# Lingeng56/conformer-pytorch-lightning

Measured on AMD Instinct MI355X. Metric: encoder frames/sec (80-d fbank, T=1000), whole job, higher is better.
Workload: dtype bf16

## Files before the change

### conformer-pytorch-lightning_amd/cfm/__init__.py

```python
import ctypes
import os
import threading

import torch

_HERE = os.path.dirname(os.path.abspath(__file__))
LIB_PATH = os.path.join(os.path.dirname(_HERE), "libconformer_gfx950.so")

F32, BF16, F16 = 0, 1, 2
ACT_NONE, ACT_SILU, ACT_RELU, ACT_GLU, ACT_DSILU, ACT_DRELU = 0, 1, 2, 3, 4, 5
TILE_AUTO_TRAIN = -1

_DT = {torch.float32: F32, torch.bfloat16: BF16, torch.float16: F16}
_TORCH_DT = {F32: torch.float32, BF16: torch.bfloat16, F16: torch.float16}

c_p = ctypes.c_void_p
c_i64 = ctypes.c_int64
c_i32 = ctypes.c_int32
c_f = ctypes.c_float


class GemmDesc(ctypes.Structure):
    _fields_ = [("A", c_p), ("W", c_p), ("W_lo", c_p), ("bias", c_p), ("residual", c_p), ("row_mask", c_p), ("C", c_p),
                ("lda", c_i64), ("ldc", c_i64), ("ldr", c_i64),
# ... 86 lines not shown
                ("p_hidden_m", ctypes.c_float), ("p_hidden", ctypes.c_float), ("p_branch", ctypes.c_float), ("p_attn", ctypes.c_float),
                ("p_attn_out", ctypes.c_float), ("seed", ctypes.c_uint32), ("deterministic", c_i32), ("grads_accumulate", c_i32),
                ("n_groups", c_i32), ("groups", ctypes.POINTER(TrainGroup)), ("defer_wgrad", c_i32)]


_TRAIN_SAVED = ["xn1", "z1", "h1", "xn2", "qkv", "ctx", "xn3", "u", "glu", "s", "xn4", "z2", "h2", "x1", "x2", "x3", "x4", "c", "lse", "stats"]
_TRAIN_SCRATCH = ["dxn", "dz", "dyb", "ds", "dglu", "du", "dctx", "dqkv", "delta", "ln_ws", "dwbn_ws", "dy_ws", "dz2", "dyb2", "dyb3", "dyb4"]
_TRAIN_GRADS = ["slab", "ln_ffm_g", "ln_ffm_b", "ln_mha_g", "ln_mha_b", "ln_conv_g", "ln_conv_b", "ln_ff_g", "ln_ff_b", "ln_final_g", "ln_final_b",
                "ffm_w1", "ffm_b1", "ffm_w2", "ffm_b2", "ff_w1", "ff_b1", "ff_w2", "ff_b2", "out_w", "out_b", "pw2_w", "pw2_b", "dw_w", "dw_b", "bn_g", "bn_b",
                "pos_bias_u", "q_bias", "qkv_row_off", "qkv_bias_off", "pw1_row_off", "pw1_bias_off", "qkv_bias_off2"]


class LayerTrainSaved(ctypes.Structure):
    _fields_ = [(n, c_p) for n in _TRAIN_SAVED]


class LayerTrainScratch(ctypes.Structure):
    _fields_ = [(n, c_p) for n in _TRAIN_SCRATCH]


class LayerTrainGrads(ctypes.Structure):
    _fields_ = [(n, c_p) for n in _TRAIN_GRADS]


class LayerWeights(ctypes.Structure):
    _fields_ = [(n, c_p) for n in _LAYER_W_FIELDS]


class CtcGroup(ctypes.Structure):
    _fields_ = [("logits", c_p), ("ld", c_i64), ("B", c_i32), ("T", c_i32), ("Umax", c_i32), ("enc_lens", c_p), ("labels", c_p), ("label_lens", c_p),
                ("work", c_p), ("alpha", c_p), ("lse", c_p), ("nll", c_p), ("nll_shifted", c_p), ("beta", c_p)]


class RnntDesc(ctypes.Structure):
    _fields_ = [("logits", c_p), ("ld", c_i64), ("logits_dtype", c_i32), ("B", c_i32), ("T", c_i32), ("U1", c_i32), ("V", c_i32), ("blank", c_i32),
                ("targets", c_p), ("logit_lens", c_p), ("target_lens", c_p),
                ("lse", c_p), ("lp_blank", c_p), ("lp_label", c_p), ("alpha", c_p), ("beta", c_p), ("shift", c_p),
                ("nll", c_p), ("nll_shifted", c_p), ("ll_alpha", c_p),
                ("grad", c_p), ("ld_grad", c_i64), ("grad_dtype", c_i32), ("grad_cols", c_i32), ("gscale", ctypes.c_float),
                ("gscale_stride", c_i32), ("gscale_dev", c_p), ("clamp", ctypes.c_float)]


class Lattice(ctypes.Structure):
    _fields_ = [("B", c_i32), ("T_max", c_i32), ("U1_max", c_i32), ("M", c_i64), ("off", c_p), ("T", c_p), ("U", c_p), ("enc_row0", c_p),
                ("pred_row0", c_p), ("n_enc", c_i64), ("n_pred", c_i64), ("blk_off", c_p)]


class RnntPackedDesc(ctypes.Structure):
    _fields_ = [("lat", Lattice), ("logits", c_p), ("ld", c_i64), ("logits_dtype", c_i32), ("V", c_i32), ("blank", c_i32), ("ld_targets", c_i32),
                ("targets", c_p), ("lse", c_p), ("lp_blank", c_p), ("lp_label", c_p), ("alpha", c_p), ("beta", c_p), ("shift", c_p),
                ("nll", c_p), ("nll_shifted", c_p), ("ll_alpha", c_p),
                ("grad", c_p), ("ld_grad", c_i64), ("grad_dtype", c_i32), ("grad_cols", c_i32), ("gscale", ctypes.c_float),
                ("gscale_stride", c_i32), ("gscale_dev", c_p), ("clamp", ctypes.c_float)]


class LnBwdDesc(ctypes.Structure):
    _fields_ = [("x", c_p), ("dy", c_p), ("gamma", c_p), ("row_mask", c_p), ("dres", c_p), ("dx", c_p), ("dgamma", c_p), ("dbeta", c_p), ("ws", c_p),
                ("dx2", c_p), ("M", c_i64), ("D", c_i32), ("dy_dtype", c_i32), ("dx2_dtype", c_i32), ("accumulate", c_i32),
                ("eps", ctypes.c_float), ("alpha2", ctypes.c_float), ("p1", ctypes.c_float), ("p2", ctypes.c_float),
                ("seed1", ctypes.c_uint32), ("seed2", ctypes.c_uint32), ("dx2_row_mask", c_p),
                ("chain_x", c_p), ("chain_gamma", c_p), ("chain_dgamma", c_p), ("chain_dbeta", c_p)]


class GreedyDesc(ctypes.Structure):
    _fields_ = [("embed", c_p), ("lstm_w", c_p * 4), ("lstm_b", c_p * 4), ("proj_w", c_p), ("proj_b", c_p), ("pf_w", c_p), ("pf_b", c_p), ("out_w", c_p),
                ("out_b", c_p), ("enc_proj", c_p), ("token", c_p), ("t", c_p), ("count", c_p), ("frame_count", c_p), ("hyps", c_p), ("lens", c_p),
                ("h", c_p), ("c", c_p), ("h_new", c_p), ("c_new", c_p), ("pred", c_p), ("act", c_p), ("pmax", c_p), ("pidx", c_p), ("done", c_p),
                ("n_done", c_p), ("hyp_cap", c_i64), ("hyp_ld", c_i64), ("B", c_i32), ("T", c_i32), ("L", c_i32), ("E", c_i32), ("H", c_i32),
                ("P", c_i32), ("J", c_i32), ("Vp", c_i32), ("blank", c_i32), ("n_steps", c_i32)]


class GreedyChunkDesc(ctypes.Structure):
    _fields_ = ([("embed", c_p), ("lstm_w", c_p * 4), ("lstm_b", c_p * 4)] +
                [(n, c_p) for n in ("proj_w", "proj_b", "pf_w", "pf_b", "out_w", "out_b", "ef_w", "ef_b", "enc", "enc_proj", "token", "t", "count", "frame_count",
                                    "hyps", "lens", "h", "c", "h_new", "c_new", "pred", "pp", "act", "pmax", "pidx", "rows", "row_off", "row_cnt", "n_rows",
                                    "steps", "overflow", "done", "n_done")] +
                [("hyp_cap", c_i64), ("hyp_ld", c_i64)] +
                [(n, c_i32) for n in ("B", "chunk", "L", "E", "H", "P", "J", "D", "Vp", "blank", "n_steps", "carry")])


class FbankDesc(ctypes.Structure):
    _fields_ = ([(n, c_p) for n in ("samples", "lengths", "feats_length", "carry_in", "carry_out", "fresh_in", "pos_in", "fresh_out", "pos_out", "twiddle", "window",
                                    "mel_w", "mel_start", "mel_len", "mel_off", "out")] + [("ld", c_i64)] +
                [(n, c_i32) for n in ("B", "n_cols", "rows", "F", "win", "shift", "padded", "mel_nnz", "samples_i16", "carry_n", "hop")] +
                [("dither", c_f), ("seed", ctypes.c_uint32)])


class FfnSplitDesc(ctypes.Structure):
    _fields_ = [("x", c_p), ("psum", c_p), ("psum_b2", c_p), ("psum_splits", c_i32), ("psum_alpha", c_f), ("ln1_g", c_p), ("ln1_b", c_p), ("ln2_g", c_p),
                ("ln2_b", c_p), ("rows_out", c_p), ("rows2_out", c_p), ("ln_g", c_p), ("ln_b", c_p), ("w1", c_p), ("b1", c_p), ("N1", c_i32), ("act", c_i32),
                ("w2", c_p), ("psum_out", c_p), ("out16", c_p), ("ldo", c_i64), ("M", c_i32), ("D", c_i32), ("mode", c_i32), ("w_dtype", c_i32), ("eps", c_f),
                ("kv_ring", c_p), ("ring_offsets", c_p), ("ring_T", c_i32), ("ring_H", c_i32), ("ring_Tq", c_i32)]


class LayerScratch(ctypes.Structure):
    _fields_ = [(n, c_p) for n in ("xn", "hid", "qkv", "pos", "ctx", "glu", "dw")] + [("psum", c_p), ("psum_splits", c_i32)]


class LayerIO(ctypes.Structure):
    _fields_ = [("B", c_i32), ("T", c_i32), ("D", c_i32), ("H", c_i32), ("FF", c_i32), ("ktaps", c_i32),
                ("act_dtype", c_i32), ("w_dtype", c_i32),
                ("attn_mask", c_p), ("am_sb", c_i64), ("am_sq", c_i64),
                ("pad_valid", c_p), ("pos_embed", c_p), ("pos_rows", c_i32),
                ("pos_proj", c_p), ("pos_proj_ld", c_i64),
                ("attn_cache", c_p), ("cache_T", c_i32), ("new_cache", c_p), ("after_g", c_p), ("after_b", c_p), ("after_out", c_p),
                ("kv_ring", c_p), ("stream_offset", c_p), ("ring_T", c_i32), ("causal_conv", c_i32), ("conv_cache", c_p), ("pos_shared", c_i32),
                ("next_w", c_p), ("next_x_out", c_p), ("macaron_done", c_i32)]


_lib = None
_lock = threading.Lock()


def lib():
    global _lib
    if _lib is not None:
        return _lib
    with _lock:
        if _lib is not None:
            return _lib
        if not os.path.exists(LIB_PATH):
            raise RuntimeError(
                "libconformer_gfx950.so not found at %s -- build it with `python -c 'import __graft_entry__ as g; g.build()'` "
                "or `make -C conformer-pytorch-lightning_amd/csrc`. There is no CPU fallback." % LIB_PATH)
        L = ctypes.CDLL(LIB_PATH)
        L.cfm_version.restype = ctypes.c_int
        L.cfm_last_error.restype = ctypes.c_char_p
        L.cfm_device_ok.restype = ctypes.c_int
        L.cfm_gemm.argtypes = [ctypes.POINTER(GemmDesc), c_p]
        L.cfm_attention.argtypes = [ctypes.POINTER(AttnDesc), c_p]
        L.cfm_ffn_fused.argtypes = [ctypes.POINTER(FfnDesc), c_p]
        L.cfm_rowchain.argtypes = [ctypes.POINTER(RowChainDesc), c_p]
        L.cfm_rowchain_supported.argtypes = [c_i32, c_i32]
        L.cfm_rowchain_pair_supported.argtypes = [c_i32, c_i32]
        L.cfm_layernorm.argtypes = [c_p, c_p, c_p, c_p, c_i32, c_p, c_p, c_p, c_i32, c_p, ctypes.c_float, c_i64, c_i32, c_p]
        L.cfm_kv_cache_pack.argtypes = [c_p, c_i32, c_p, c_p, c_i32, c_i64, c_i64, c_i64, c_i64, c_p, c_i32, c_i32, c_i32, c_i32, c_p]
        L.cfm_dwconv_bn_silu.argtypes = [c_p, c_i32, c_p, c_p, c_p, c_p, c_p, c_i32, c_i32, c_i32, c_i32, c_i32, c_p]
        L.cfm_conv1_relu.argtypes = [c_p, c_p, c_p, c_p, c_i32, c_i32, c_i32, c_i32, c_i32, c_p, c_p, c_p]
        L.cfm_conv1_relu_mma.argtypes = [c_p, c_p, c_p, c_p, c_i32, c_i32, c_i32, c_i32, c_i32, c_p, c_p, c_p]
        L.cfm_conv12_supported.argtypes = [c_i32, c_i32]
        L.cfm_pack_matrices.argtypes = [c_p, c_i32, c_i64, c_i32, c_i32, c_p]
        L.cfm_pack_vectors.argtypes = [c_p, c_p, c_p, c_i64, c_p]
        L.cfm_greedy_step.argtypes = [ctypes.POINTER(GreedyDesc), c_p]
        L.cfm_greedy_chunk_begin.argtypes = [ctypes.POINTER(GreedyChunkDesc), c_p]
        L.cfm_greedy_chunk_step.argtypes = [ctypes.POINTER(GreedyChunkDesc), c_p]
        L.cfm_fbank.argtypes = [ctypes.POINTER(FbankDesc), c_p]
        L.cfm_fbank_stream.argtypes = [ctypes.POINTER(FbankDesc), c_p]
        L.cfm_ffn_split.argtypes = [ctypes.POINTER(FfnSplitDesc), c_p]
        L.cfm_ffn_split_supported.argtypes = [c_i32, c_i32]
        L.cfm_attention_bwd_force_general.argtypes = [c_i32]
        L.cfm_attention_bwd_force_general.restype = None
        L.cfm_set_cin_merge.argtypes = [c_i32]
        L.cfm_set_cin_merge.restype = c_i32
        L.cfm_dwconv_bn_train_bwd_acc.argtypes = [c_p, c_i32, c_p, c_p, c_p, c_i32, c_p, c_p, c_i32, c_p, c_p, c_p, c_p, c_p, c_p, c_i32, c_i32, c_i32, c_i32, c_i32, c_p]
        L.cfm_layernorm_bwd_fused.argtypes = [ctypes.POINTER(LnBwdDesc), c_p]
        L.cfm_conv12_relu.argtypes = [c_p, c_p, c_p, c_p, c_p, c_p, c_i32, c_i32, c_i32, c_i32, c_i32, c_p, c_p, c_p]
        L.cfm_valid_mask.argtypes = [c_p, c_i32, c_p, c_i32, c_i32, c_i32, c_i32, c_p]
        L.cfm_chunk_mask.argtypes = [c_p, c_i32, c_i32, c_i32, c_p]
        L.cfm_attn_mask.argtypes = [c_p, c_p, c_p, c_i32, c_i32, c_p]
        L.cfm_cast.argtypes = [c_p, c_i32, c_p, c_i32, c_i64, c_p]
        L.cfm_add_rows.argtypes = [c_p, c_p, c_i64, c_i32, c_i32, c_p]
        L.cfm_encoder_layer_forward.argtypes = [ctypes.POINTER(LayerWeights), ctypes.POINTER(LayerScratch),
                                                ctypes.POINTER(LayerIO), c_p, c_p, c_i32, c_p, c_p, c_p]
        L.cfm_ctc_nll.argtypes = [c_p, c_i64, c_i32, c_i32, c_i32, c_p, c_p, c_i32, c_p, c_p, c_p, c_p]
        L.cfm_joint_act.argtypes = [c_p, c_i64, c_p, c_i64, c_p, c_i32, c_i32, c_i32, c_i32, c_i32, c_p]
        L.cfm_joint_act_bwd.argtypes = [c_p, c_i64, c_p, c_i64, c_p, c_p, c_p, c_p, c_i32, c_i32, c_i32, c_i32, c_p]
        L.cfm_joint_act_bwd_ws.argtypes = [c_i32, c_i32, c_i32, c_i32]
        L.cfm_rnnt_nll.argtypes = [ctypes.POINTER(RnntDesc), c_p]
        L.cfm_rnnt_grad.argtypes = [ctypes.POINTER(RnntDesc), c_p]
        L.cfm_rnnt_packed_nll.argtypes = [ctypes.POINTER(RnntPackedDesc), c_p]
        L.cfm_rnnt_packed_grad.argtypes = [ctypes.POINTER(RnntPackedDesc), c_p]
        L.cfm_joint_act_packed.argtypes = [c_p, c_i64, c_p, c_i64, c_p, c_i32, ctypes.POINTER(Lattice), c_i32, c_p]
        L.cfm_joint_act_packed_bwd.argtypes = [c_p, c_i64, c_p, c_i64, c_p, c_p, c_p, c_p, ctypes.POINTER(Lattice), c_i32, c_p]
        c_f = ctypes.c_float
        L.cfm_gemm_tn.argtypes = [ctypes.POINTER(GemmTnDesc), c_p]
        L.cfm_gemm_tn_group.argtypes = [ctypes.POINTER(GemmTnDesc), c_i32, c_p]
        L.cfm_attention_bwd.argtypes = [ctypes.POINTER(AttnBwdDesc), c_p]
        L.cfm_layernorm_bwd_ws.argtypes = [c_i64, c_i32]
        L.cfm_layernorm_bwd.argtypes = [c_p, c_p, c_i32, c_p, c_p, c_p, c_p, c_p, c_p, c_p, c_f, c_i64, c_i32, c_p]
        L.cfm_glu_bwd.argtypes = [c_p, c_i32, c_p, c_i32, c_p, c_i32, c_i64, c_i32, c_p]
        L.cfm_dwconv_bn_ws.argtypes = [c_i32, c_i32, c_i32]
        L.cfm_dwconv_bn_train.argtypes = [c_p, c_i32, c_p, c_p, c_p, c_p, c_p, c_p, c_f, c_f, c_p, c_p, c_p, c_i32, c_p, c_i32, c_i32, c_i32, c_i32, c_p]
        L.cfm_dwconv_bn_train_bwd.argtypes = [c_p, c_i32, c_p, c_p, c_p, c_i32, c_p, c_p, c_i32, c_p, c_p, c_p, c_p, c_p, c_p, c_i32, c_i32, c_i32, c_i32, c_p]
        L.cfm_col2im_relu_bwd.argtypes = [c_p, c_i32, c_p, c_i32, c_p, c_i32, c_i32, c_i32, c_i32, c_i32, c_p]
        L.cfm_conv1_wgrad_ws.argtypes = [c_i32, c_i32, c_i32]
        L.cfm_conv1_wgrad.argtypes = [c_p, c_i32, c_p, c_p, c_p, c_p, c_p, c_p, c_i32, c_i32, c_i32, c_i32, c_p]
        L.cfm_ctc_nll_train_groups.argtypes = [ctypes.POINTER(CtcGroup), c_i32, c_i32, c_p]
        L.cfm_ctc_grad.argtypes = [c_p, c_i64, c_i32, c_i32, c_i32, c_p, c_p, c_i32, c_p, c_p, c_p, c_p, c_p, c_p, c_f, c_p, c_p, c_p]
        L.cfm_adam_step.argtypes = [c_p, c_p, c_p, c_p, c_i64, c_f, c_f, c_f, c_f, c_f, c_i64, c_p, c_p]
        L.cfm_sumsq.argtypes = [c_p, c_i64, c_p, c_i32, c_p, c_p]
        L.cfm_adam_clip_step.argtypes = [c_p, c_p, c_p, c_p, c_i64, c_f, c_f, c_f, c_f, c_f, c_i64, c_p, c_f, c_f, c_i32, c_p, c_p]
        L.cfm_dropout_rows.argtypes = [c_p, c_i32, c_p, c_i32, c_p, c_f, c_f, ctypes.c_uint32, c_f, ctypes.c_uint32, c_i64, c_i32, c_p]
        L.cfm_dropout_mask.argtypes = [c_p, c_i64, c_f, ctypes.c_uint32, c_p]
        L.cfm_encoder_train_forward.argtypes = [c_i32, ctypes.POINTER(LayerTrainWeights), ctypes.POINTER(LayerTrainIO), ctypes.POINTER(LayerTrainSaved),
                                                ctypes.POINTER(LayerTrainScratch), ctypes.POINTER(c_p), c_p]
        L.cfm_encoder_train_backward.argtypes = [c_i32, ctypes.POINTER(LayerTrainWeights), ctypes.POINTER(LayerTrainIO), ctypes.POINTER(LayerTrainSaved),
                                                 ctypes.POINTER(LayerTrainScratch), ctypes.POINTER(LayerTrainGrads), ctypes.POINTER(c_p), c_p, c_p, c_p,
                                                 LAYER_DONE_FN, c_p, ctypes.POINTER(c_p), c_p]
        L.cfm_stream_prep.argtypes = [c_p, c_i32, c_i32, c_i32, c_i32, c_p, c_i32, c_i32, c_p, c_p, c_p, c_p]
        L.cfm_kv_ring_write.argtypes = [c_p, c_p, c_i32, c_i64, c_i64, c_i64, c_i64, c_p, c_p, c_i32, c_i32, c_i32, c_i32, c_i32, c_p]
        L.cfm_stream_advance.argtypes = [c_p, c_p, c_i32, c_i32, c_p]
        L.cfm_dwconv_causal_bn_silu.argtypes = [c_p, c_i32, c_p, c_p, c_p, c_p, c_p, c_p, c_i32, c_i32, c_i32, c_i32, c_i32, c_p]
        L.cfm_conv_cache_update.argtypes = [c_p, c_i32, c_p, c_i32, c_i32, c_i32, c_i32, c_p]
        for name in ("cfm_layernorm_bwd_ws", "cfm_dwconv_bn_ws", "cfm_conv1_wgrad_ws", "cfm_joint_act_bwd_ws"):
            getattr(L, name).restype = c_i64
        L.cfm_prof_enable.argtypes = [c_i32]
        L.cfm_prof_enable.restype = None
        L.cfm_prof_reset.restype = None
        L.cfm_prof_collect.restype = ctypes.c_int
        L.cfm_prof_entry.argtypes = [c_i32, ctypes.c_char_p, c_i32, ctypes.POINTER(c_i64), ctypes.POINTER(ctypes.c_double),
                                     ctypes.POINTER(ctypes.c_double), ctypes.POINTER(ctypes.c_double)]
        for name in ("cfm_gemm", "cfm_ffn_fused", "cfm_rowchain", "cfm_rowchain_supported", "cfm_attention", "cfm_layernorm", "cfm_kv_cache_pack", "cfm_dwconv_bn_silu", "cfm_conv1_relu", "cfm_conv1_relu_mma", "cfm_conv12_relu", "cfm_conv12_supported",
                     "cfm_valid_mask", "cfm_chunk_mask", "cfm_attn_mask", "cfm_cast", "cfm_add_rows",
                     "cfm_encoder_layer_forward", "cfm_ctc_nll", "cfm_joint_act", "cfm_joint_act_bwd", "cfm_rnnt_nll", "cfm_rnnt_grad", "cfm_prof_entry", "cfm_gemm_tn", "cfm_gemm_tn_group", "cfm_attention_bwd",
                     "cfm_layernorm_bwd", "cfm_glu_bwd", "cfm_dwconv_bn_train", "cfm_dwconv_bn_train_bwd", "cfm_col2im_relu_bwd", "cfm_conv1_wgrad",
                     "cfm_ctc_nll_train_groups", "cfm_ctc_grad", "cfm_adam_step", "cfm_adam_clip_step", "cfm_sumsq", "cfm_dropout_rows", "cfm_dropout_mask", "cfm_pack_matrices", "cfm_pack_vectors", "cfm_greedy_step", "cfm_greedy_chunk_begin", "cfm_greedy_chunk_step", "cfm_fbank", "cfm_fbank_stream", "cfm_ffn_split", "cfm_ffn_split_supported", "cfm_layernorm_bwd_fused", "cfm_dwconv_bn_train_bwd_acc",
                     "cfm_encoder_train_forward", "cfm_encoder_train_backward", "cfm_stream_prep", "cfm_kv_ring_write", "cfm_stream_advance", "cfm_dwconv_causal_bn_silu", "cfm_conv_cache_update"):
            getattr(L, name).restype = ctypes.c_int
        _lib = L
    return _lib


def check(rc, what):
    if rc != 0:
        raise RuntimeError("%s failed (status %d): %s" % (what, rc, lib().cfm_last_error().decode(errors="replace")))


def dt_code(t):
    try:
        return _DT[t.dtype if isinstance(t, torch.Tensor) else t]
    except KeyError:
        raise TypeError("cfm: unsupported dtype %s (float32, bfloat16, float16 only)" % (t.dtype if isinstance(t, torch.Tensor) else t))


def torch_dtype(code):
    return _TORCH_DT[code]


def require_hip(*tensors):
    for t in tensors:
        if t is None:
            continue
        if not t.is_cuda:
            raise RuntimeError("cfm: tensor on %s -- this framework runs on MI355X (HIP) only; there is no CPU path" % t.device)


def ptr(t):
    return None if t is None else t.data_ptr()


def stream():
    return torch.cuda.current_stream().cuda_stream


class Precision:

    def __init__(self, name):
        if name not in ("bf16", "fp16", "fp32"):
            raise ValueError("precision must be bf16, fp16 or fp32, got %r" % (name,))
        self.name = name
        self.split = name == "fp32"
        self.w_code = F16 if name == "fp16" else BF16
        self.act_code = F32 if self.split else self.w_code
        self.w_dtype = torch_dtype(self.w_code)
        self.act_dtype = torch_dtype(self.act_code)

    def __repr__(self):
        return "Precision(%s)" % self.name


_precision = Precision(os.environ.get("CFM_PRECISION", "bf16"))


def set_precision(name):
    global _precision
    _precision = name if isinstance(name, Precision) else Precision(name)
    return _precision


def get_precision():
    return _precision


def resolve_precision(module=None):
    p = getattr(module, "precision", None) if module is not None else None
    if p is None:
        return _precision
    return p if isinstance(p, Precision) else Precision(p)


_warned = set()


def check_mode(module, what):
    if module.training:
        return True
    if torch.is_grad_enabled() and what not in _warned and any(q.requires_grad for q in module.parameters()):
        _warned.add(what)
        import warnings
        warnings.warn("%s: eval-mode forward runs inference kernels; its output is detached from the parameters. "
                      "Call .train() for a differentiable forward, or wrap inference in torch.no_grad()." % what)
    return False


from .ops import *
```

### conformer-pytorch-lightning_amd/csrc/frontend.hip

```cpp
#include <string>
#include <type_traits>

#include "cfm_common.h"

namespace {

typedef unsigned int u32x2_a4 __attribute__((ext_vector_type(2), aligned(4)));

#define CFM_INL __attribute__((always_inline))

struct Conv12Args {
    const float* x;
    const float* w1;
    const float* b1;
    const u16* W;
    const float* b2;
    u16* y;
    const float* cm_mean;
    const float* cm_istd;
    int T, F, C, T2, F2, M;
    int m_begin, m_end;
};

template <typename HT, int FM>
__global__ __launch_bounds__(512) void cfm_conv12_kernel(const Conv12Args g) {
    constexpr int BM = 32 * FM, BN = 256, BK = 64;
    constexpr int OPA = BM * (BK / 8), OPW = BN * (BK / 8);
    constexpr int BUF = OPA + OPW;
    constexpr int FN = 4;
    constexpr int NU = 2 * FM;
    constexpr int U = (NU + 7) / 8;
    __shared__ u32x4 smem[2 * BUF + 1024];
    u32x2* const w1tab = (u32x2*)(smem + 2 * BUF);

    const int tid = threadIdx.x, lane = tid & 63;
    const int wave = __builtin_amdgcn_readfirstlane(tid >> 6);
    const int wr = wave >> 2, wc = wave & 3;
    const int l15 = lane & 15, kg = lane >> 4;
    const int m0 = g.m_begin + blockIdx.x * BM;
    const int n0 = blockIdx.y * BN;
    const int N = g.C, K = 9 * g.C;
    const int slabs = g.C >> 6;

    for (int e = tid; e < slabs * 4 * 64; e += 512) {
        const int ln = e & 63, j = (e >> 6) & 3, cs = e >> 8;
        const int r = ln & 15, q = ln >> 4;
        const int ch = cs * 64 + 16 * (r >> 2) + 4 * j + (r & 3);
        u32x2 v = (u32x2){0u, 0u};
        if (q < 3) {
            const float a = g.w1[(3 * q) * g.C + ch], b = g.w1[(3 * q + 1) * g.C + ch], c = g.w1[(3 * q + 2) * g.C + ch];
            v.x = pack2<HT>(a, b);
            v.y = pack2<HT>(c, 0.f);
        } else {
            const float bv = g.b1[ch];
            const float hi = HT::to_f32(HT::from_f32(bv));
            v.x = pack2<HT>(hi, bv - hi);
        }
        w1tab[e] = v;
    }

    unsigned w_off[4];
#pragma unroll
    for (int i = 0; i < 4; ++i) {
        const int r = (i * 8 + wave) * 8 + (lane >> 3);
        const int c = (lane & 7) ^ ((r >> 1) & 7);
        const int n = n0 + r < N ? n0 + r : N - 1;
        w_off[i] = ((unsigned)n * (unsigned)K + c * 8) * 2u;
    }
    auto stageW = [&](int buf, int kt) CFM_INL {
        const unsigned kw = (unsigned)(kt * BK) * 2u;
        u32x4* const Ws = smem + buf * BUF + OPA;
#pragma unroll
        for (int i = 0; i < 4; ++i)
            __builtin_amdgcn_global_load_lds((const __attribute__((address_space(1))) void*)((const char*)g.W + (w_off[i] + kw)),
                                             (__attribute__((address_space(3))) void*)(Ws + (i * 8 + wave) * 64), 16, 0, 0);
    };

    int xbase[U], fcol[U];
#pragma unroll
    for (int ui = 0; ui < U; ++ui) {
        const int u = wave + 8 * ui;
        int m = m0 + u * 16 + l15;
        m = m < g.M ? m : g.M - 1;
        const int per_b = g.T2 * g.F2;
        const int b = m / per_b;
        const int q = m - b * per_b;
        const int t2 = q / g.F2;
        const int f2 = q - t2 * g.F2;
        fcol[ui] = 4 * f2;
        xbase[ui] = (b * g.T + 4 * t2 + (kg < 3 ? kg : 0)) * g.F + 4 * f2;
    }
    float xraw[U][3];
    auto fetch = [&](int tap) CFM_INL {
        const int dt = tap / 3, df = tap - 3 * dt;
#pragma unroll
        for (int ui = 0; ui < U; ++ui) {
            const float* xr = g.x + (xbase[ui] + 2 * dt * g.F + 2 * df);
            float v0 = xr[0], v1 = xr[1], v2 = xr[2];
            if (g.cm_mean) {
                const int f = fcol[ui] + 2 * df;
                v0 -= g.cm_mean[f]; v1 -= g.cm_mean[f + 1]; v2 -= g.cm_mean[f + 2];
                if (g.cm_istd) { v0 *= g.cm_istd[f]; v1 *= g.cm_istd[f + 1]; v2 *= g.cm_istd[f + 2]; }
            }
            xraw[ui][0] = v0; xraw[ui][1] = v1; xraw[ui][2] = v2;
        }
    };
    u32x4 xcur[U];
    auto convert = [&]() CFM_INL {
#pragma unroll
        for (int ui = 0; ui < U; ++ui) {
            xcur[ui] = (u32x4){0u, 0u, 0u, 0u};
            if (kg < 3) {
                xcur[ui].x = pack2<HT>(xraw[ui][0], xraw[ui][1]);
                xcur[ui].y = pack2<HT>(xraw[ui][2], 0.f);
            } else {
                xcur[ui].x = pack2<HT>(1.0f, 1.0f);
            }
        }
    };
    const f32x4 zero4 = (f32x4){0.f, 0.f, 0.f, 0.f};
    auto produce = [&](int buf, int cs) CFM_INL {
        u32x4* const As = smem + buf * BUF;
        u32x4 wf[4];
#pragma unroll
        for (int j = 0; j < 4; ++j) {
            const u32x2 t = w1tab[(cs * 4 + j) * 64 + lane];
            wf[j] = (u32x4){t.x, t.y, 0u, 0u};
        }
#pragma unroll
        for (int ui = 0; ui < U; ++ui) {
            const int u = wave + 8 * ui;
            if (u < NU) {
                f32x4 a[4];
#pragma unroll
                for (int j = 0; j < 4; ++j) {
                    a[j] = HT::mfma(wf[j], xcur[ui], zero4);
                    a[j].x = fmaxf(a[j].x, 0.f); a[j].y = fmaxf(a[j].y, 0.f); a[j].z = fmaxf(a[j].z, 0.f); a[j].w = fmaxf(a[j].w, 0.f);
                }
                const int row = u * 16 + l15;
                const int sw = (row >> 1) & 7;
                As[row * 8 + ((2 * kg) ^ sw)] = pack8<HT>(a[0], a[1]);
                As[row * 8 + ((2 * kg + 1) ^ sw)] = pack8<HT>(a[2], a[3]);
            }
        }
    };

    f32x4 acc[FM][FN];
#pragma unroll
    for (int i = 0; i < FM; ++i)
#pragma unroll
        for (int j = 0; j < FN; ++j) acc[i][j] = zero4;
    const int sw = (lane >> 1) & 7;
    const int a_row = wr * (16 * FM) + l15, w_row = wc * 64 + l15;
    auto compute = [&](int buf) CFM_INL {
        const u32x4* const As = smem + buf * BUF;
        const u32x4* const Ws = As + OPA;
#pragma unroll
        for (int kk = 0; kk < BK / 32; ++kk) {
            const int c = (kk * 4 + kg) ^ sw;
            u32x4 af[FM], wf[FN];
#pragma unroll
            for (int j = 0; j < FN; ++j) wf[j] = Ws[(w_row + j * 16) * 8 + c];
#pragma unroll
            for (int i = 0; i < FM; ++i) af[i] = As[(a_row + i * 16) * 8 + c];
            __builtin_amdgcn_s_setprio(1);
#pragma unroll
            for (int i = 0; i < FM; ++i)
#pragma unroll
                for (int j = 0; j < FN; ++j) acc[i][j] = HT::mfma(wf[j], af[i], acc[i][j]);
            __builtin_amdgcn_s_setprio(0);
        }
    };

    fetch(0);
    stageW(0, 0);
    convert();
    fetch(1);
    __syncthreads();
    produce(0, 0);
    const int q4 = kg * 4;
    f32x4 bias_r[FN];
#pragma unroll
    for (int j = 0; j < FN; ++j) {
        const int col = n0 + wc * 64 + j * 16 + q4;
        bias_r[j] = col + 3 < N ? *(const f32x4*)(g.b2 + col) : zero4;
    }
    __syncthreads();
    for (int tap = 0; tap < 9; ++tap) {
#pragma unroll
        for (int cs = 0; cs < 8; ++cs) {
            if (cs < slabs) {
                const int kt = tap * slabs + cs;
                const int cur = kt & 1;
                const bool last_slab = cs == slabs - 1;
                if (!(tap == 8 && last_slab)) {
                    stageW(cur ^ 1, kt + 1);
                    if (!last_slab) {
                        produce(cur ^ 1, cs + 1);
                    } else {
                        convert();
                        if (tap + 2 < 9) fetch(tap + 2);
                        produce(cur ^ 1, 0);
                    }
                }
                compute(cur);
                __syncthreads();
            }
        }
    }

    const int col0 = n0 + wc * 64 + q4;
#pragma unroll
    for (int i = 0; i < FM; ++i) {
        const int row = m0 + wr * (16 * FM) + i * 16 + l15;
        u16* const rowp = g.y + ((int64_t)row * g.C + col0);
#pragma unroll
        for (int j = 0; j < FN; ++j) {
            f32x4 v = acc[i][j] + bias_r[j];
            v.x = fmaxf(v.x, 0.f); v.y = fmaxf(v.y, 0.f); v.z = fmaxf(v.z, 0.f); v.w = fmaxf(v.w, 0.f);
            if (row < g.m_end && col0 + j * 16 + 3 < N) *(u32x2_a4*)(rowp + j * 16) = (u32x2){pack2<HT>(v.x, v.y), pack2<HT>(v.z, v.w)};
        }
    }
}

template <typename HT, int FM>
int launch(const Conv12Args& a, hipStream_t s, const char* name) {
    const int rows = a.m_end - a.m_begin, BM = 32 * FM;
    const int tiles = (rows + BM - 1) / BM, nh = (a.C + 255) / 256;
    CfmProfScope prof(name, s, 2.0 * rows * (double)a.C * (9.0 * a.C + 32.0 * nh), (double)rows * a.C * 2 + 9.0 * a.C * a.C * 2);
    CFM_LAUNCH((cfm_conv12_kernel<HT, FM>), dim3(tiles, nh), dim3(512), 0, s, a);
    return cfm_launch_status(name);
}

template <typename HT>
int run(Conv12Args a, int cus, hipStream_t s, const char* nm_big, const char* nm_tail) {
    const int M = a.M;
    cus /= (a.C + 255) / 256;
    const int whole = (M / (256 * cus)) * cus;
    int rest = M - whole * 256;
    if (rest > 0 && rest > 128 * cus) {
        a.m_begin = 0; a.m_end = M;
        return launch<HT, 8>(a, s, nm_big);
    }
    if (whole > 0) {
        a.m_begin = 0; a.m_end = whole * 256;
        if (int rc = launch<HT, 8>(a, s, nm_big)) return rc;
    }
    if (rest > 0) {
        a.m_begin = whole * 256; a.m_end = M;
        if (rest <= 64 * cus) return launch<HT, 2>(a, s, nm_tail);
        if (rest <= 96 * cus) return launch<HT, 3>(a, s, nm_tail);
        return launch<HT, 4>(a, s, nm_tail);
    }
    return CFM_OK;
}

int num_cus() {
    static int n = 0;
    if (n == 0) {
        int dev = 0;
        hipDeviceProp_t prop;
        n = (hipGetDevice(&dev) == hipSuccess && hipGetDeviceProperties(&prop, dev) == hipSuccess && prop.multiProcessorCount > 0) ? prop.multiProcessorCount : 256;
    }
    return n;
}

}

extern "C" int cfm_conv12_supported(int32_t C, int32_t y_dtype) { return C % 64 == 0 && C >= 64 && (C <= 256 || C == 512) && cfm_is16(y_dtype); }

extern "C" int cfm_conv12_relu(const float* x, const float* w1, const float* b1, const void* w2, const float* b2, void* y, int32_t y_dtype, int32_t B,
                               int32_t T, int32_t F, int32_t C, const float* cmvn_mean, const float* cmvn_istd, cfm_stream_t stream) {
    CFM_CHECK_ARG(x && w1 && b1 && w2 && b2 && y, "cfm_conv12_relu: null pointer");
    CFM_CHECK_ARG(cfm_conv12_supported(C, y_dtype), "cfm_conv12_relu: C must be 64, 128, 192, 256 or 512 and y 16-bit (the type its products are rounded to)");
    const int T1 = (T - 3) / 2 + 1, F1 = (F - 3) / 2 + 1;
    const int T2 = (T1 - 3) / 2 + 1, F2 = (F1 - 3) / 2 + 1;
    CFM_CHECK_ARG(B > 0 && T >= 7 && F >= 7 && T2 >= 1 && F2 >= 1, "cfm_conv12_relu: the input is shorter than two 3x3 stride-2 windows");
    CFM_CHECK_ARG(!cmvn_istd || cmvn_mean, "cfm_conv12_relu: cmvn_istd without cmvn_mean");
    const int64_t M = (int64_t)B * T2 * F2;
    CFM_CHECK_ARG((int64_t)B * T * F < ((int64_t)1 << 31) && M * C < ((int64_t)1 << 31), "cfm_conv12_relu: 32-bit element offsets");
    Conv12Args a;
    a.x = x; a.w1 = w1; a.b1 = b1; a.W = (const u16*)w2; a.b2 = b2; a.y = (u16*)y; a.cm_mean = cmvn_mean; a.cm_istd = cmvn_istd;
    a.T = T; a.F = F; a.C = C; a.T2 = T2; a.F2 = F2; a.M = (int)M; a.m_begin = 0; a.m_end = (int)M;
    hipStream_t s = (hipStream_t)stream;
    if (y_dtype == CFM_BF16) return run<BF16>(a, num_cus(), s, "conv12_bf16_256", "conv12_bf16_tail");
    return run<F16>(a, num_cus(), s, "conv12_f16_256", "conv12_f16_tail");
}
```

### include/cfm.h

```cpp
#ifndef CFM_H_
#define CFM_H_

#include <stddef.h>
#include <stdint.h>

#ifdef __cplusplus
extern "C" {
#endif

#define CFM_VERSION 305

typedef void* cfm_stream_t;

typedef enum { CFM_F32 = 0, CFM_BF16 = 1, CFM_F16 = 2 } cfm_dtype;

typedef enum {
    CFM_OK = 0,
    CFM_ERR_ARG = -1,
    CFM_ERR_LAUNCH = -2,
    CFM_ERR_UNSUPPORTED = -3
} cfm_status;

typedef enum {
    CFM_ACT_NONE = 0, CFM_ACT_SILU = 1, CFM_ACT_RELU = 2, CFM_ACT_GLU = 3,
// ... 13 lines not shown
    const float* residual;
    const uint8_t* row_mask;
    void* C;
    int64_t lda, ldc, ldr;
    int32_t M, N, K;
    int32_t a_dtype, w_dtype, c_dtype;
    int32_t act;
    float alpha;
    int32_t conv_C, conv_T1, conv_F1, conv_T2, conv_F2;
    int32_t tile;
    int32_t mask_mode;
    void* C_pre;
    int64_t ld_pre;
    int32_t pre_dtype;
    int32_t aux_dtype;
    const void* aux;
    int64_t ld_aux;
    float drop_p, drop2_p;
    uint32_t drop_seed, drop2_seed;
} cfm_gemm_desc;

int cfm_gemm(const cfm_gemm_desc* d, cfm_stream_t stream);

typedef struct {
    const void* A;
    const void* B;
    float* C;
    float* colsum;
    const uint8_t* row_mask;
    int64_t lda, ldb, ldc;
    int32_t M, N, K;
    int32_t a_dtype, b_dtype, mma_dtype;
    int32_t split, accumulate, splits;
    float alpha;
    int32_t conv_C, conv_T1, conv_F1, conv_T2, conv_F2;
    const int64_t* row_off;
    const int64_t* colsum_off;
    int32_t tile;
    const int64_t* colsum_off2;
} cfm_gemm_tn_desc;

int cfm_gemm_tn(const cfm_gemm_tn_desc* d, cfm_stream_t stream);
int cfm_gemm_tn_group(const cfm_gemm_tn_desc* descs, int32_t n, cfm_stream_t stream);

typedef struct {
    const float* x;
    const float *ln_g, *ln_b;
    const void *w1f, *w2f;
    const float *b1, *b2;
    const float *ln1_g, *ln1_b, *ln2_g, *ln2_b;
    float* out_f32;
    void* out16;
    int64_t M;
    int32_t D, FF;
    int32_t w_dtype, out16_dtype;
    int32_t act;
    int32_t add_x;
    float alpha, eps;
} cfm_ffn_desc;

int cfm_ffn_fused(const cfm_ffn_desc* d, cfm_stream_t stream);

typedef struct {
    const float* x;
    const void* head_a;
    const void* head_w;
    const float* head_b;
    const float* head_res;
    const uint8_t* head_mask;
    const float *ln_g, *ln_b;
    const uint8_t* ln_mask;
    const void *w1f, *w2n;
    const float *b1, *b2;
    const float *ln1_g, *ln1_b, *ln2_g, *ln2_b;
    float* out_f32;
    void* out16;
    const void* tail_w;
    const float* tail_b;
    void* tail_out;
    int64_t M;
    int32_t D, FF, tail_N, tail_glu;
    int32_t w_dtype;
    float alpha, eps;
    float* out2_f32;
    const float *dw_w, *dw_b, *dw_scale, *dw_shift;
    int32_t dw_T, dw_K;
    const float *s2_ln_g, *s2_ln_b;
    const void *s2_w1f, *s2_w2n;
    const float *s2_b1, *s2_b2;
    float* s2_out_f32;
    float s2_alpha;
    float* psum_out;
    const float* psum_in;
    const float* psum_b2;
    float psum_alpha;
    const void *cin_a, *cin_w;
    const float *cin_b, *cin_res;
    float* cin_out;
    const float *cin_ln_g, *cin_ln_b;
    const uint8_t* cin_mask;
    const void* cin_tail_w;
    const float* cin_tail_b;
    int32_t tail_pair;
} cfm_rowchain_desc;

int cfm_rowchain(const cfm_rowchain_desc* d, cfm_stream_t stream);
int cfm_rowchain_supported(int32_t D, int32_t FF);
int cfm_rowchain_dw_supported(int32_t D);
int cfm_rowchain_pair_supported(int32_t D, int32_t FF);

int cfm_layernorm(const float* x, const float* g1, const float* b1, void* out1, int out1_dtype,
                  const float* g2, const float* b2, void* out2, int out2_dtype,
                  const uint8_t* row_mask, float eps, int64_t M, int32_t D, cfm_stream_t stream);

typedef struct {
    const void* q;
    const void* k;
    const void* v;
    const void* p;
    const float* bias_u;
    const float* bias_v;
    const uint8_t* mask;
    void* out;
    int64_t q_sb, q_st, k_sb, k_st, k_sh, v_sb, v_st, v_sh, p_sb, p_st, m_sb, m_sq;
    int32_t B, H, Tq, Tk, dk;
    int32_t q_dtype, kv_dtype, p_dtype, out_dtype, mma_dtype;
    int32_t split;
    float scale;
    float* lse;
    float drop_p;
    uint32_t drop_seed;
} cfm_attn_desc;

int cfm_attention(const cfm_attn_desc* d, cfm_stream_t stream);
int cfm_attention_group(const cfm_attn_desc* descs, int32_t n, cfm_stream_t stream);

int cfm_kv_cache_pack(const float* old_cache, int32_t Tc, const void* k, const void* v, int32_t kv_dtype,
                      int64_t k_sb, int64_t k_st, int64_t v_sb, int64_t v_st, float* new_cache,
                      int32_t B, int32_t H, int32_t Tn, int32_t dk, cfm_stream_t stream);

int cfm_dwconv_bn_silu(const void* x, int x_dtype, const float* w, const float* dw_bias,
                       const float* bn_scale, const float* bn_shift, void* y, int y_dtype, int32_t B,
                       int32_t T, int32_t D, int32_t ktaps, cfm_stream_t stream);

int cfm_conv1_relu(const float* x, const float* w, const float* bias, void* y, int y_dtype, int32_t B,
                   int32_t T, int32_t F, int32_t C, const float* cmvn_mean, const float* cmvn_istd, cfm_stream_t stream);

int cfm_conv1_relu_mma(const float* x, const float* w, const float* bias, void* y, int y_dtype, int32_t B, int32_t T, int32_t F,
                       int32_t C, const float* cmvn_mean, const float* cmvn_istd, cfm_stream_t stream);

int cfm_conv12_supported(int32_t C, int32_t y_dtype);
int cfm_conv12_relu(const float* x, const float* w1, const float* b1, const void* w2, const float* b2, void* y, int32_t y_dtype, int32_t B,
                    int32_t T, int32_t F, int32_t C, const float* cmvn_mean, const float* cmvn_istd, cfm_stream_t stream);

int cfm_valid_mask(const void* lengths, int len_is_i64, uint8_t* out, int32_t B, int32_t T, int32_t first,
                   int32_t stride, cfm_stream_t stream);
int cfm_chunk_mask(uint8_t* out, int32_t size, int32_t chunk, int32_t left, cfm_stream_t stream);
int cfm_attn_mask(const uint8_t* valid, const uint8_t* chunk, uint8_t* out, int32_t B, int32_t T,
                  cfm_stream_t stream);

int cfm_stream_prep(const int32_t* offsets, int32_t B, int32_t T, int32_t need, int32_t ring_T, const float* pe, int32_t max_len, int32_t D,
                    uint8_t* slot_mask, float* pos_rows, float* abs_rows, cfm_stream_t stream);
int cfm_kv_ring_write(const void* k, const void* v, int32_t kv_dtype, int64_t k_sb, int64_t k_st, int64_t v_sb, int64_t v_st, float* ring,
                      const int32_t* offsets, int32_t B, int32_t H, int32_t T, int32_t dk, int32_t ring_T, cfm_stream_t stream);
int cfm_stream_advance(int32_t* offsets, const uint8_t* active, int32_t B, int32_t T, cfm_stream_t stream);
int cfm_dwconv_causal_bn_silu(const void* x, int32_t x_dtype, const float* cache, const float* w, const float* dw_bias, const float* bn_scale,
                              const float* bn_shift, void* y, int32_t y_dtype, int32_t B, int32_t T, int32_t D, int32_t ktaps, cfm_stream_t stream);
int cfm_conv_cache_update(const void* x, int32_t x_dtype, float* cache, int32_t B, int32_t T, int32_t D, int32_t ktaps, cfm_stream_t stream);

int cfm_cast(const void* src, int src_dtype, void* dst, int dst_dtype, int64_t n, cfm_stream_t stream);
int cfm_add_rows(float* x, const float* add, int64_t rows, int32_t D, int32_t group, cfm_stream_t stream);

typedef struct {
    const float *ln_ffm_g, *ln_ffm_b, *ln_mha_g, *ln_mha_b, *ln_conv_g, *ln_conv_b, *ln_ff_g, *ln_ff_b,
        *ln_final_g, *ln_final_b;
    const void *ffm_w1, *ffm_w1_lo, *ffm_w2, *ffm_w2_lo;
    const float *ffm_b1, *ffm_b2;
    const void *ff_w1, *ff_w1_lo, *ff_w2, *ff_w2_lo;
    const float *ff_b1, *ff_b2;
    const void *ffm_w1f, *ffm_w2f, *ff_w1f, *ff_w2f;
    const void *ffm_w2n, *ff_w2n;
    const void *qkv_wf, *out_wf, *pw1_wf, *pw2_wf;
    const void *qkv_w, *qkv_w_lo, *pos_w, *pos_w_lo, *out_w, *out_w_lo;
    const float *qkv_b, *out_b, *bias_u, *bias_v;
    const void *pw1_w, *pw1_w_lo, *pw2_w, *pw2_w_lo;
    const float *pw1_b, *pw2_b, *dw_w, *dw_b, *bn_scale, *bn_shift;
} cfm_layer_weights;

typedef struct {
    void *xn, *hid, *qkv, *pos, *ctx, *glu, *dw;
    float* psum;
    int32_t psum_splits;
} cfm_layer_scratch;
#define CFM_PAIR_MAX_ROWS 4096
#define CFM_FFSPLIT_MAX_ROWS 1536

typedef struct {
    int32_t B, T, D, H, FF, ktaps;
    int32_t act_dtype;
    int32_t w_dtype;
    const uint8_t* attn_mask;
    int64_t am_sb, am_sq;
    const uint8_t* pad_valid;
    const float* pos_embed;
    int32_t pos_rows;
    const void* pos_proj;
    int64_t pos_proj_ld;
    const float* attn_cache;
    int32_t cache_T;
    float* new_cache;
    const float *after_g, *after_b;
    float* after_out;
    float* kv_ring;
    const int32_t* stream_offset;
    int32_t ring_T;
    int32_t causal_conv;
    float* conv_cache;
    int32_t pos_shared;
    const cfm_layer_weights* next_w;
    float* next_x_out;
    int32_t macaron_done;
} cfm_layer_io;

int cfm_encoder_layer_forward(const cfm_layer_weights* w, const cfm_layer_scratch* s, const cfm_layer_io* io,
                              const float* x_in, float* x_out, int xn_ready, const float* next_g,
                              const float* next_b, cfm_stream_t stream);

int cfm_ctc_nll(const float* logits, int64_t ld, int32_t B, int32_t T, int32_t V, const int32_t* enc_lens,
                const int32_t* labels, int32_t Umax, const int32_t* label_lens, float* work, float* nll, cfm_stream_t stream);

int cfm_joint_act(const float* enc, int64_t ld_e, const float* pred, int64_t ld_p, void* out, int32_t out_dtype, int32_t B,
                  int32_t T, int32_t U, int32_t J, cfm_stream_t stream);

typedef struct {
    const void* logits;
    int64_t ld;
    int32_t logits_dtype;
    int32_t B, T, U1, V, blank;
    const int32_t* targets;
    const int32_t* logit_lens;
    const int32_t* target_lens;
    float *lse, *lp_blank, *lp_label, *alpha, *beta, *shift;
    float *nll, *nll_shifted, *ll_alpha;
    void* grad;
    int64_t ld_grad;
    int32_t grad_dtype, grad_cols;
    float gscale;
    int32_t gscale_stride;
    const float* gscale_dev;
    float clamp;
} cfm_rnnt_desc;
int cfm_rnnt_nll(const cfm_rnnt_desc* d, cfm_stream_t stream);
int cfm_rnnt_grad(const cfm_rnnt_desc* d, cfm_stream_t stream);

int64_t cfm_joint_act_bwd_ws(int32_t B, int32_t T, int32_t U, int32_t J);
int cfm_joint_act_bwd(const float* enc, int64_t ld_e, const float* pred, int64_t ld_p, const float* dact, float* d_enc, float* d_pred,
                      float* work, int32_t B, int32_t T, int32_t U, int32_t J, cfm_stream_t stream);

typedef struct {
    int32_t B, T_max, U1_max;
    int64_t M;
    const int64_t* off;
    const int32_t* T;
    const int32_t* U;
    const int64_t* enc_row0;
    const int64_t* pred_row0;
    int64_t n_enc, n_pred;
    const int64_t* blk_off;
} cfm_lattice;

int cfm_joint_act_packed(const float* enc, int64_t ld_e, const float* pred, int64_t ld_p, void* out, int32_t out_dtype, const cfm_lattice* lat,
                         int32_t J, cfm_stream_t stream);
int cfm_joint_act_packed_bwd(const float* enc, int64_t ld_e, const float* pred, int64_t ld_p, const float* dact, float* d_enc, float* d_pred,
                             float* work, const cfm_lattice* lat, int32_t J, cfm_stream_t stream);

typedef struct {
    cfm_lattice lat;
    const void* logits;
    int64_t ld;
    int32_t logits_dtype, V, blank, ld_targets;
    const int32_t* targets;
    float *lse, *lp_blank, *lp_label, *alpha, *beta, *shift;
    float *nll, *nll_shifted, *ll_alpha;
    void* grad;
    int64_t ld_grad;
    int32_t grad_dtype, grad_cols;
    float gscale;
    int32_t gscale_stride;
    const float* gscale_dev;
    float clamp;
} cfm_rnnt_packed_desc;
int cfm_rnnt_packed_nll(const cfm_rnnt_packed_desc* d, cfm_stream_t stream);
int cfm_rnnt_packed_grad(const cfm_rnnt_packed_desc* d, cfm_stream_t stream);

int64_t cfm_layernorm_bwd_ws(int64_t M, int32_t D);
typedef struct {
    const float* x;
    const void* dy;
    const float* gamma;
    const uint8_t* row_mask;
    const float* dres;
    float *dx, *dgamma, *dbeta, *ws;
    void* dx2;
    int64_t M;
    int32_t D, dy_dtype, dx2_dtype, accumulate;
    float eps, alpha2, p1, p2;
// ... 241 lines not shown
```

Before: 26.61 million.

## Add 320-row conv12 tile with cost-model tile planner

Adds an FM=10 (320-row) instantiation of the fused conv1+conv2 subsampling kernel. It handles the odd half-unit of A-fragment production, reloads A fragments in groups of five to limit register pressure, and defers the bias load past the main loop. A simple launch/step cost model now picks between the existing 256-row-plus-tail split and a single 320-row launch, aiming to cut wave-quantization waste on the CU count. The larger tile raises register and LDS pressure, and the cost-model constants are hand-fitted.

```diff
diff --git a/conformer-pytorch-lightning_amd/cfm/__init__.py b/conformer-pytorch-lightning_amd/cfm/__init__.py
--- a/conformer-pytorch-lightning_amd/cfm/__init__.py
+++ b/conformer-pytorch-lightning_amd/cfm/__init__.py
@@ -262,6 +262,9 @@
         L.cfm_attention_bwd_force_general.restype = None
         L.cfm_set_cin_merge.argtypes = [c_i32]
         L.cfm_set_cin_merge.restype = c_i32
+        L.cfm_set_conv12_tile.argtypes = [c_i32]
+        L.cfm_set_conv12_tile.restype = c_i32
+        L.cfm_conv12_plan.argtypes = [c_i64, c_i32, c_i32, ctypes.POINTER(c_i32), ctypes.POINTER(c_i32)]
         L.cfm_dwconv_bn_train_bwd_acc.argtypes = [c_p, c_i32, c_p, c_p, c_p, c_i32, c_p, c_p, c_i32, c_p, c_p, c_p, c_p, c_p, c_p, c_i32, c_i32, c_i32, c_i32, c_i32, c_p]
         L.cfm_layernorm_bwd_fused.argtypes = [ctypes.POINTER(LnBwdDesc), c_p]
         L.cfm_conv12_relu.argtypes = [c_p, c_p, c_p, c_p, c_p, c_p, c_i32, c_i32, c_i32, c_i32, c_i32, c_p, c_p, c_p]
diff --git a/conformer-pytorch-lightning_amd/csrc/frontend.hip b/conformer-pytorch-lightning_amd/csrc/frontend.hip
--- a/conformer-pytorch-lightning_amd/csrc/frontend.hip
+++ b/conformer-pytorch-lightning_amd/csrc/frontend.hip
@@ -30,6 +30,9 @@
     constexpr int FN = 4;
     constexpr int NU = 2 * FM;
     constexpr int U = (NU + 7) / 8;
+    constexpr bool HALF = NU > 8 && NU % 8 == 4;
+    constexpr int G = FM > 8 ? 5 : FM;
+    static_assert(FM % G == 0, "A-fragment groups");
     __shared__ u32x4 smem[2 * BUF + 1024];
     u32x2* const w1tab = (u32x2*)(smem + 2 * BUF);
 
@@ -79,7 +82,7 @@
     int xbase[U], fcol[U];
 #pragma unroll
     for (int ui = 0; ui < U; ++ui) {
-        const int u = wave + 8 * ui;
+        const int u = HALF && ui == U - 1 ? 8 * ui + (wave & 3) : wave + 8 * ui;
         int m = m0 + u * 16 + l15;
         m = m < g.M ? m : g.M - 1;
         const int per_b = g.T2 * g.F2;
@@ -129,6 +132,18 @@
         }
 #pragma unroll
         for (int ui = 0; ui < U; ++ui) {
+            if (HALF && ui == U - 1) {
+                const int u = 8 * ui + (wave & 3), h = wave >> 2;
+                f32x4 a[2];
+#pragma unroll
+                for (int j = 0; j < 2; ++j) {
+                    a[j] = HT::mfma(h ? wf[2 + j] : wf[j], xcur[ui], zero4);
+                    a[j].x = fmaxf(a[j].x, 0.f); a[j].y = fmaxf(a[j].y, 0.f); a[j].z = fmaxf(a[j].z, 0.f); a[j].w = fmaxf(a[j].w, 0.f);
+                }
+                const int row = u * 16 + l15;
+                As[row * 8 + ((2 * kg + h) ^ ((row >> 1) & 7))] = pack8<HT>(a[0], a[1]);
+                continue;
+            }
             const int u = wave + 8 * ui;
             if (u < NU) {
                 f32x4 a[4];
@@ -158,16 +173,21 @@
 #pragma unroll
         for (int kk = 0; kk < BK / 32; ++kk) {
             const int c = (kk * 4 + kg) ^ sw;
-            u32x4 af[FM], wf[FN];
+            u32x4 af[G], wf[FN];
 #pragma unroll
             for (int j = 0; j < FN; ++j) wf[j] = Ws[(w_row + j * 16) * 8 + c];
 #pragma unroll
-            for (int i = 0; i < FM; ++i) af[i] = As[(a_row + i * 16) * 8 + c];
+            for (int i = 0; i < G; ++i) af[i] = As[(a_row + i * 16) * 8 + c];
             __builtin_amdgcn_s_setprio(1);
 #pragma unroll
-            for (int i = 0; i < FM; ++i)
-#pragma unroll
-                for (int j = 0; j < FN; ++j) acc[i][j] = HT::mfma(wf[j], af[i], acc[i][j]);
+            for (int i0 = 0; i0 < FM; i0 += G) {
+#pragma unroll
+                for (int i = 0; i < G; ++i) {
+#pragma unroll
+                    for (int j = 0; j < FN; ++j) acc[i0 + i][j] = HT::mfma(wf[j], af[i], acc[i0 + i][j]);
+                    if (i0 + G < FM) af[i] = As[(a_row + (i0 + G + i) * 16) * 8 + c];
+                }
+            }
             __builtin_amdgcn_s_setprio(0);
         }
     };
@@ -180,10 +200,12 @@
     produce(0, 0);
     const int q4 = kg * 4;
     f32x4 bias_r[FN];
-#pragma unroll
-    for (int j = 0; j < FN; ++j) {
-        const int col = n0 + wc * 64 + j * 16 + q4;
-        bias_r[j] = col + 3 < N ? *(const f32x4*)(g.b2 + col) : zero4;
+    if constexpr (FM <= 8) {
+#pragma unroll
+        for (int j = 0; j < FN; ++j) {
+            const int col = n0 + wc * 64 + j * 16 + q4;
+            bias_r[j] = col + 3 < N ? *(const f32x4*)(g.b2 + col) : zero4;
+        }
     }
     __syncthreads();
     for (int tap = 0; tap < 9; ++tap) {
@@ -209,6 +231,13 @@
         }
     }
 
+    if constexpr (FM > 8) {
+#pragma unroll
+        for (int j = 0; j < FN; ++j) {
+            const int col = n0 + wc * 64 + j * 16 + q4;
+            bias_r[j] = col + 3 < N ? *(const f32x4*)(g.b2 + col) : zero4;
+        }
+    }
     const int col0 = n0 + wc * 64 + q4;
 #pragma unroll
     for (int i = 0; i < FM; ++i) {
@@ -232,25 +261,57 @@
     return cfm_launch_status(name);
 }
 
+constexpr double CONV12_LAUNCH = 4.0, CONV12_STEP_FIXED = 0.46, CONV12_STEP_PER_FM = 0.219;
+
+struct Conv12Plan {
+    int fm_main, fm_tail;
+    int64_t rows_main;
+};
+
+double conv12_cost(int64_t rows, int fm, int cus, int C) {
+    if (rows <= 0) return 0.0;
+    const int64_t tiles = (rows + 32 * fm - 1) / (32 * fm);
+    return CONV12_LAUNCH + (double)((tiles + cus - 1) / cus) * (9.0 * C / 64.0) * (CONV12_STEP_FIXED + CONV12_STEP_PER_FM * fm);
+}
+
+Conv12Plan conv12_plan(int64_t M, int C, int cus, int force_fm) {
+    cus /= (C + 255) / 256;
+    if (cus < 1) cus = 1;
+    if (force_fm > 0) return Conv12Plan{force_fm, 0, M};
+    const int64_t whole = (M / (256 * (int64_t)cus)) * cus;
+    const int64_t rest = M - whole * 256;
+    Conv12Plan split{whole > 0 ? 8 : 0, 0, whole * 256};
+    if (rest > 128 * (int64_t)cus) split = Conv12Plan{8, 0, M};
+    else if (rest > 0) split.fm_tail = rest <= 64 * (int64_t)cus ? 2 : rest <= 96 * (int64_t)cus ? 3 : 4;
+    const double c_split = conv12_cost(split.rows_main, split.fm_main, cus, C) + conv12_cost(M - split.rows_main, split.fm_tail, cus, C);
+    if (conv12_cost(M, 10, cus, C) < c_split) return Conv12Plan{10, 0, M};
+    return split;
+}
+
+int g_conv12_tile = 0;
+
 template <typename HT>
-int run(Conv12Args a, int cus, hipStream_t s, const char* nm_big, const char* nm_tail) {
-    const int M = a.M;
-    cus /= (a.C + 255) / 256;
-    const int whole = (M / (256 * cus)) * cus;
-    int rest = M - whole * 256;
-    if (rest > 0 && rest > 128 * cus) {
-        a.m_begin = 0; a.m_end = M;
-        return launch<HT, 8>(a, s, nm_big);
-    }
-    if (whole > 0) {
-        a.m_begin = 0; a.m_end = whole * 256;
-        if (int rc = launch<HT, 8>(a, s, nm_big)) return rc;
-    }
-    if (rest > 0) {
-        a.m_begin = whole * 256; a.m_end = M;
-        if (rest <= 64 * cus) return launch<HT, 2>(a, s, nm_tail);
-        if (rest <= 96 * cus) return launch<HT, 3>(a, s, nm_tail);
-        return launch<HT, 4>(a, s, nm_tail);
+int launch_fm(int fm, const Conv12Args& a, hipStream_t s, const char* const* nm) {
+    switch (fm) {
+        case 2: return launch<HT, 2>(a, s, nm[1]);
+        case 3: return launch<HT, 3>(a, s, nm[1]);
+        case 4: return launch<HT, 4>(a, s, nm[1]);
+        case 8: return launch<HT, 8>(a, s, nm[0]);
+        case 10: return launch<HT, 10>(a, s, nm[2]);
+    }
+    return cfm_fail(CFM_ERR_ARG, "cfm_conv12_relu: no such tile");
+}
+
+template <typename HT>
+int run(Conv12Args a, int cus, hipStream_t s, const char* const* nm) {
+    const Conv12Plan p = conv12_plan(a.M, a.C, cus, g_conv12_tile);
+    if (p.fm_main) {
+        a.m_begin = 0; a.m_end = (int)p.rows_main;
+        if (int rc = launch_fm<HT>(p.fm_main, a, s, nm)) return rc;
+    }
+    if (p.fm_tail) {
+        a.m_begin = (int)p.rows_main; a.m_end = a.M;
+        return launch_fm<HT>(p.fm_tail, a, s, nm);
     }
     return CFM_OK;
 }
@@ -283,6 +344,21 @@
     a.x = x; a.w1 = w1; a.b1 = b1; a.W = (const u16*)w2; a.b2 = b2; a.y = (u16*)y; a.cm_mean = cmvn_mean; a.cm_istd = cmvn_istd;
     a.T = T; a.F = F; a.C = C; a.T2 = T2; a.F2 = F2; a.M = (int)M; a.m_begin = 0; a.m_end = (int)M;
     hipStream_t s = (hipStream_t)stream;
-    if (y_dtype == CFM_BF16) return run<BF16>(a, num_cus(), s, "conv12_bf16_256", "conv12_bf16_tail");
-    return run<F16>(a, num_cus(), s, "conv12_f16_256", "conv12_f16_tail");
-}
+    static const char* const nm_bf16[3] = {"conv12_bf16_256", "conv12_bf16_tail", "conv12_bf16_320"};
+    static const char* const nm_f16[3] = {"conv12_f16_256", "conv12_f16_tail", "conv12_f16_320"};
+    if (y_dtype == CFM_BF16) return run<BF16>(a, num_cus(), s, nm_bf16);
+    return run<F16>(a, num_cus(), s, nm_f16);
+}
+
+extern "C" int32_t cfm_set_conv12_tile(int32_t fm) {
+    const int prev = g_conv12_tile;
+    if (fm == 0 || fm == 2 || fm == 3 || fm == 4 || fm == 8 || fm == 10) g_conv12_tile = fm;
+    return prev;
+}
+
+extern "C" int cfm_conv12_plan(int64_t M, int32_t C, int32_t cus, int32_t* fm_main, int32_t* fm_tail) {
+    CFM_CHECK_ARG(M > 0 && cus > 0 && fm_main && fm_tail && C >= 64, "cfm_conv12_plan: bad argument");
+    const Conv12Plan p = conv12_plan(M, C, cus, 0);
+    *fm_main = p.fm_main; *fm_tail = p.fm_tail;
+    return CFM_OK;
+}
diff --git a/include/cfm.h b/include/cfm.h
--- a/include/cfm.h
+++ b/include/cfm.h
@@ -189,6 +189,8 @@
 int cfm_conv12_supported(int32_t C, int32_t y_dtype);
 int cfm_conv12_relu(const float* x, const float* w1, const float* b1, const void* w2, const float* b2, void* y, int32_t y_dtype, int32_t B,
                     int32_t T, int32_t F, int32_t C, const float* cmvn_mean, const float* cmvn_istd, cfm_stream_t stream);
+int cfm_conv12_plan(int64_t M, int32_t C, int32_t cus, int32_t* fm_main, int32_t* fm_tail);
+int32_t cfm_set_conv12_tile(int32_t fm);
 
 int cfm_valid_mask(const void* lengths, int len_is_i64, uint8_t* out, int32_t B, int32_t T, int32_t first,
                    int32_t stride, cfm_stream_t stream);
```

After: 26.97 million, median of 6. +1.4%, better.
